# DaehwanKimLab/hisat-genotype

Hardware: AMD Instinct MI355X
Metric: typed reads/sec at HLA-A (~7k alleles, 2x150bp) (higher is better)
Workload: dtype u64 bitsets, f64 EM

## Files before the change

### hisat-genotype_amd/csrc/hgx_common.hpp

```cpp
#pragma once
#include <hip/hip_runtime.h>

#include <cstdint>
#include <cstring>
#include <cstdio>
#include <mutex>
#include <string>
#include <vector>

#include "hgx.h"

extern "C" void hgx_set_error(const char *fmt, ...);
extern "C" const char *hgx_test_switch(const char *name);
static inline bool hgx_switch_has(const char *name, const char *token) {
    const char *v = hgx_test_switch(name);
    if (!v) return false;
    const size_t n = strlen(token);
    for (const char *p = v;;) {
        const char *e = strchr(p, ',');
        const size_t len = e ? (size_t)(e - p) : strlen(p);
        if (len == n && memcmp(p, token, n) == 0) return true;
        if (!e) return false;
        p = e + 1;
    }
// ... 32 lines not shown
    uint64_t *d_exon_mask, *d_gene_mask;
    int pat_state = 0;
    uint16_t *d_pid = nullptr;
    uint32_t *d_vals = nullptr;
    int32_t *d_nval = nullptr;
    int pat_dmax = 0;
    std::mutex *pat_mu = nullptr;
};
#define HGX_PAT_D 512

struct hgx_classes {
    int32_t n_classes, a_pad, w64, c64;
    uint64_t *d_bits;
    int64_t *d_count;
    int64_t *d_first_row;
    uint64_t *d_bitsT;
    int32_t n_act = -1, a1p = 0;
    int32_t *d_act = nullptr;
    uint64_t *d_bitsC = nullptr;
    uint64_t *d_bitsTC = nullptr;
    int32_t *h_act = nullptr;
    int32_t *h_rank = nullptr;
    uint64_t *d_wrow = nullptr, *d_wcol = nullptr;
    void *d_setup0 = nullptr, *d_setup1 = nullptr;
    hipStream_t made_on = nullptr;
    hipEvent_t ready = nullptr;
    void *d_keep[12] = {nullptr, nullptr, nullptr, nullptr, nullptr, nullptr, nullptr, nullptr,
                        nullptr, nullptr, nullptr, nullptr};
};

// ... 55 lines not shown

int hgx_ensure_transposed(hgx_classes *c, hipStream_t st);
int hgx_pair_classes_sel(const hgx_index *ix, const uint64_t *compat, const int32_t *pair_off, const uint32_t *refs,
                         const int64_t *sel, int32_t n_pairs, uint64_t *eb, uint64_t *gb, uint64_t *eh,
                         uint64_t *gh, hipStream_t st);

struct hgx_groups;
int hgx_group_pairs_seg(hgx_groups **out, const int32_t *pair_off, const uint32_t *refs, int32_t n_pairs, int32_t level,
                        const uint32_t *pair_seg, void *stream);
int hgx_level_classes_grouped_seg(hgx_classes **out, const hgx_index *ix, const uint64_t *compat, const int32_t *pair_off,
                                  const uint32_t *refs, hgx_groups *g, uint64_t *rows_scratch, uint64_t *hash_scratch,
                                  const uint32_t *pair_seg, void *stream);
int hgx_dedup_classes_seg(hgx_classes **out, const uint64_t *rows, const uint64_t *row_hash, int64_t n_rows, int32_t a_pad,
                          const uint32_t *row_seg, void *stream);

int hgx_pair_classes_fused_launch(const hgx_index *ix, const uint64_t *compat, const int32_t *pair_off, const uint32_t *refs,
                                  int32_t n_pairs, int32_t level, unsigned long long *keys, uint32_t tmask, uint32_t *rep,
                                  uint32_t *slot_of, int *bad, uint64_t *rows, hipStream_t st);

int hgx_scan_u32_dev(const uint32_t *in, uint32_t *out, long n, void *scratch, uint32_t *total_dev, hipStream_t st);
size_t hgx_scan_u32_scratch_bytes(long n);
void hgx_front_set_last(int route, int decline, long long bytes);

int hgx_pair_classes_dedup_ev(hgx_classes **out, const hgx_index *ix, const uint64_t *compat, const int32_t *pair_off, const uint32_t *refs,
                              int32_t n_pairs, int32_t level, uint64_t *rows_scratch, void *stream, void *ev_begin, void *ev_end);

#define HGX_EMPTY_KEY 0xFFFFFFFFFFFFFFFFull

__device__ __forceinline__ uint64_t mix64(uint64_t x) {
    x ^= x >> 30; x *= 0xbf58476d1ce4e5b9ull;
// ... 70 lines not shown
```

### hisat-genotype_amd/csrc/hgx_counts.hip

```cpp
#include <algorithm>
#include <cstdint>
#include <vector>

#include <hip/hip_runtime.h>

#include "hgx_common.hpp"

namespace {
__device__ __forceinline__ uint64_t lane_u64(uint64_t v, int l) {
    return ((uint64_t)(uint32_t)__builtin_amdgcn_readlane((int)(v >> 32), l) << 32) | (uint32_t)__builtin_amdgcn_readlane((int)v, l);
}
}

__global__ __launch_bounds__(256) void k_first_set_rows(const uint64_t *__restrict__ BT, int n_rows, int c64, int32_t *__restrict__ first) {
    const int lane = threadIdx.x & 63;
    const long row = ((long)blockIdx.x * blockDim.x + threadIdx.x) >> 6;
    if (row >= n_rows) return;
    int best = 0x7fffffff;
    for (int w0 = 0; w0 < c64; w0 += 64) {
        const int w = w0 + lane;
        const uint64_t x = w < c64 ? BT[(size_t)row * c64 + w] : 0ull;
        const uint64_t hit = __ballot(x != 0ull);
        if (hit) {
            const int l = __builtin_ctzll(hit);
// ... 35 lines not shown
    hipStream_t st = (hipStream_t)stream;
    DevBuf b_a, b_f;
    ALLOC(b_a, (size_t)n * 4); ALLOC(b_f, (size_t)n * 4);
    { int rc_ = hgx_h2d(b_a.p, alleles_host, (size_t)n * 4, st); if (rc_) return rc_; }
    hipLaunchKernelGGL(k_first_classes, dim3(n), dim3(256), 0, st, c->d_bits, c->n_classes, c->w64, b_a.as<int32_t>(), b_f.as<int32_t>());
    HIPCHK(hipGetLastError());
    { int rc_ = hgx_d2h(first_host, b_f.p, (size_t)n * 4, st); if (rc_) return rc_; }
    { int rc_ = hgx_sync(st); if (rc_) return rc_; }
    return HGX_OK;
}

constexpr int AC_WAVES = 4;
__global__ __launch_bounds__(64 * AC_WAVES) void k_allele_counts_direct(const uint64_t *__restrict__ bits, int C, int w64,
                                                                         const int64_t *__restrict__ count, int per_wave,
                                                                         unsigned long long *__restrict__ cnt_part,
                                                                         int *__restrict__ first_part, int A) {
    __shared__ int s_first[AC_WAVES][32][64];
    __shared__ uint32_t s_cnt[AC_WAVES][32][64];
    const int lane = threadIdx.x & 63, wv = threadIdx.x >> 6;
    const int n_half = 2 * w64;
    const int hw = blockIdx.x * 64 + lane;
    const bool live = hw < n_half;
    const int c0 = (blockIdx.y * AC_WAVES + wv) * per_wave, c1 = min(C, c0 + per_wave);
    const uint32_t *rows = (const uint32_t *)bits;
    uint32_t acc[32];
#pragma unroll
    for (int b = 0; b < 32; ++b) { acc[b] = 0u; s_first[wv][b][lane] = 0x7fffffff; }
    uint32_t seen = 0u;
    constexpr int U = 8;
    uint32_t xn[U], nn[U];
    auto fetch = [&](int cb) {
#pragma unroll
        for (int u = 0; u < U; ++u) {
            const int c = cb + u;
            xn[u] = (live && c < c1) ? rows[(size_t)c * n_half + hw] : 0u;
            nn[u] = c < c1 ? (uint32_t)count[c] : 0u;
        }
    };
// ... 20 lines not shown
            }
        }
    }
#pragma unroll
    for (int b = 0; b < 32; ++b) s_cnt[wv][b][lane] = acc[b];
    __syncthreads();
    if (live) {
#pragma unroll
        for (int k = 0; k < 32 / AC_WAVES; ++k) {
            const int b = wv * (32 / AC_WAVES) + k;
            unsigned long long t = 0ull;
            int f = 0x7fffffff;
#pragma unroll
            for (int q = 0; q < AC_WAVES; ++q) { t += (unsigned long long)s_cnt[q][b][lane]; f = min(f, s_first[q][b][lane]); }
            const int a = hw * 32 + b;
            cnt_part[(size_t)blockIdx.y * A + a] = t;
            first_part[(size_t)blockIdx.y * A + a] = f;
        }
    }
}
__global__ void k_allele_counts_reduce(const unsigned long long *__restrict__ cnt_part, const int *__restrict__ first_part, int groups,
                                       int A, int64_t *__restrict__ cnt, int *__restrict__ first) {
    const int a = blockIdx.x * blockDim.x + threadIdx.x;
    if (a >= A) return;
    unsigned long long t = 0ull;
    int f = 0x7fffffff;
    for (int g0 = 0; g0 < groups; g0 += 8) {
        unsigned long long tv[8];
        int fv[8];
#pragma unroll
        for (int k = 0; k < 8; ++k) {
            const bool in = g0 + k < groups;
// ... 33 lines not shown
            m &= m - 1;
            if (cls >= n_classes) break;
            sum += count[cls];
            if (first < 0) first = cls;
        }
    }
    out_count[a] = sum;
    out_first[a] = first;
}

extern "C" int hgx_allele_counts_on(const hgx_classes *cc, int64_t *count_host, int32_t *first_host, void *stream);
extern "C" int hgx_allele_counts(const hgx_classes *cc, int64_t *count_host, int32_t *first_host) {
    return hgx_allele_counts_on(cc, count_host, first_host, nullptr);
}
extern "C" int hgx_allele_counts_on(const hgx_classes *cc, int64_t *count_host, int32_t *first_host, void *stream) {
    ARGCHK(cc && count_host && first_host);
    hipStream_t st = (hipStream_t)stream;
    hgx_classes_order_after(cc, st);
    hgx_classes *c = const_cast<hgx_classes *>(cc);
    const int A = c->a_pad;
    if (c->n_classes == 0) {
        for (int a = 0; a < A; ++a) { count_host[a] = 0; first_host[a] = -1; }
        return HGX_OK;
    }
    {
        const int C = c->n_classes;
        DevBuf b_cnt, b_first, b_big, b_cp, b_fp;
        ALLOC(b_cnt, (size_t)A * 8); ALLOC(b_first, (size_t)A * 4); ALLOC(b_big, 16);
        HIPCHK(hipMemsetAsync(b_big.p, 0, 16, st));
        hipLaunchKernelGGL(k_allele_counts_check, dim3(nblk(C, 256 * 16)), dim3(256), 0, st, c->d_count, C, b_big.as<unsigned long long>());
        const int spans = (2 * c->w64 + 63) / 64;
        const int groups = std::max(1, std::min(256 / std::max(spans, 1), (C + 64 * AC_WAVES - 1) / (64 * AC_WAVES)));
        const int per_wave = (C + groups * AC_WAVES - 1) / (groups * AC_WAVES);
        ALLOC(b_cp, (size_t)groups * A * 8); ALLOC(b_fp, (size_t)groups * A * 4);
        hipLaunchKernelGGL(k_allele_counts_direct, dim3(spans, groups), dim3(64 * AC_WAVES), 0, st, c->d_bits, C, c->w64, c->d_count,
                           per_wave, b_cp.as<unsigned long long>(), b_fp.as<int>(), A);
        hipLaunchKernelGGL(k_allele_counts_reduce, dim3(nblk(A, 64)), dim3(64), 0, st, b_cp.as<unsigned long long>(), b_fp.as<int>(),
                           groups, A, b_cnt.as<int64_t>(), b_first.as<int>());
        HIPCHK(hipGetLastError());
        unsigned long long big[2] = {0, 0};
        { int rc_ = hgx_d2h(count_host, b_cnt.p, (size_t)A * 8, st); if (rc_) return rc_; }
        { int rc_ = hgx_d2h(first_host, b_first.p, (size_t)A * 4, st); if (rc_) return rc_; }
        { int rc_ = hgx_d2h(big, b_big.p, 16, st); if (rc_) return rc_; }
        { int rc_ = hgx_sync(st); if (rc_) return rc_; }
        if (!big[0] && big[1] < (1ull << 32)) return HGX_OK;
    }
    int rc = hgx_ensure_transposed(c, st);
    if (rc) return rc;
    DevBuf b_c, b_i;
    ALLOC(b_c, (size_t)A * 8); ALLOC(b_i, (size_t)A * 4);
    hipLaunchKernelGGL(k_allele_counts_wide, dim3(nblk(A, 256)), dim3(256), 0, st, c->d_bitsT, A, c->c64, c->n_classes, c->d_count,
// ... 9 lines not shown
```

### hisat-genotype_amd/csrc/hgx_dedup.hip

```cpp
#include <algorithm>
#include <vector>

#include "hgx_common.hpp"


__global__ __launch_bounds__(256) void k_hash_rows(const uint64_t *__restrict__ rows, long n_rows, int w64,
                                                   const uint64_t *__restrict__ mask, uint64_t *__restrict__ hash) {
    const int lane = threadIdx.x & 63;
    const long row = ((long)blockIdx.x * blockDim.x + threadIdx.x) >> 6;
    if (row >= n_rows) return;
    uint64_t h = 0;
    bool nz = false;
    for (int w = lane; w < w64; w += 64) {
        uint64_t x = rows[(size_t)row * w64 + w];
        if (mask) x &= mask[w];
        h += word_hash(x, w);
        nz = nz || x != 0;
    }
    h = wave_sum_u64(h);
    const bool any_nz = __any(nz);
    if (lane == 0) hash[row] = finish_hash(h, any_nz);
}

#define SCAN_T 1024
// ... 132 lines not shown
        h = (h + 1) & tmask;
    }
}

__device__ __forceinline__ uint64_t readlane_u64(uint64_t v, int l) {
    const uint32_t lo = (uint32_t)__builtin_amdgcn_readlane((int)v, l), hi = (uint32_t)__builtin_amdgcn_readlane((int)(v >> 32), l);
    return ((uint64_t)hi << 32) | lo;
}
__device__ __forceinline__ uint64_t shfl_u64(uint64_t v, int l) {
    const uint32_t lo = __shfl((uint32_t)v, l, 64), hi = __shfl((uint32_t)(v >> 32), l, 64);
    return ((uint64_t)hi << 32) | lo;
}

template <int BS, int RPT>
__global__ __launch_bounds__(BS) void k_ht_insert(const uint64_t *__restrict__ hash, const int64_t *__restrict__ weight, long n,
                                                    unsigned long long *__restrict__ keys, uint32_t *__restrict__ first,
                                                    unsigned long long *__restrict__ cnt, uint32_t tmask,
                                                    uint32_t *__restrict__ slot_of) {
    constexpr int ROWS = BS * RPT, SLOTS = 2 * ROWS, SPT = SLOTS / BS;
    __shared__ unsigned long long lkey[SLOTS], lcnt[SLOTS];
    __shared__ uint32_t lmin[SLOTS];
    __shared__ uint8_t wtab[BS / 64][256];
    const int tid = threadIdx.x, lane = tid & 63;
    for (int s = tid; s < SLOTS; s += BS) { lkey[s] = HGX_EMPTY_KEY; lcnt[s] = 0; lmin[s] = HT_NONE; }
    const long base = (long)blockIdx.x * ROWS;
    uint64_t key[RPT];
    unsigned long long w[RPT];
#pragma unroll
    for (int r = 0; r < RPT; ++r) {
        const long i = base + (long)r * BS + tid;
        key[r] = i < n ? hash[i] : HGX_EMPTY_KEY;
        w[r] = weight && i < n ? (unsigned long long)weight[i] : 1ull;
    }
    __syncthreads();
    volatile uint8_t *wt = wtab[tid >> 6];
    uint32_t ls[RPT];
#pragma unroll
    for (int r = 0; r < RPT; ++r) {
        const bool valid = key[r] != HGX_EMPTY_KEY;
        const uint32_t bucket = (uint32_t)(key[r] >> 24) & 255u;
// ... 85 lines not shown
                          uint32_t *__restrict__ is_first) {
    const long s = (long)blockIdx.x * blockDim.x + threadIdx.x;
    if (s < T && keys[s] != HGX_EMPTY_KEY) is_first[first[s]] = 1u;
}
__global__ void k_ht_finalize(const unsigned long long *__restrict__ keys, const uint32_t *__restrict__ first,
                              const unsigned long long *__restrict__ cnt, long T, const uint32_t *__restrict__ rank,
                              int64_t *__restrict__ out_first, int64_t *__restrict__ out_count) {
    const long s = (long)blockIdx.x * blockDim.x + threadIdx.x;
    if (s >= T || keys[s] == HGX_EMPTY_KEY) return;
    const uint32_t c = rank[first[s]];
    out_first[c] = (int64_t)first[s];
    out_count[c] = (int64_t)cnt[s];
}
__global__ __launch_bounds__(256) void k_verify_ht(const uint64_t *__restrict__ rows, int w64, const uint64_t *__restrict__ mask,
                                                   const uint32_t *__restrict__ slot_of, const uint32_t *__restrict__ first, long n,
                                                   uint32_t *__restrict__ is_first,
                                                   int *__restrict__ bad, uint32_t *__restrict__ bad_rows = nullptr,
                                                   uint32_t *__restrict__ n_bad = nullptr, const uint32_t *__restrict__ seg = nullptr) {
    constexpr int R = 4;
    const int lane = threadIdx.x & 63;
    const long r0 = (((long)blockIdx.x * blockDim.x + threadIdx.x) >> 6) * R;
    if (r0 >= n) return;
    uint32_t sl[R], h[R];
#pragma unroll
    for (int k = 0; k < R; ++k) sl[k] = r0 + k < n ? slot_of[r0 + k] : HT_NONE;
#pragma unroll
    for (int k = 0; k < R; ++k) h[k] = sl[k] != HT_NONE ? first[sl[k]] : 0u;
    if (lane < R && r0 + lane < n) {
        uint32_t fl = 0;
#pragma unroll
        for (int k = 0; k < R; ++k)
            if (lane == k) fl = sl[k] != HT_NONE && h[k] == (uint32_t)(r0 + k) ? 1u : 0u;
        is_first[r0 + lane] = fl;
    }
    typedef unsigned long long u64x2 __attribute__((ext_vector_type(2)));
    const u64x2 *m = (const u64x2 *)mask;
// ... 108 lines not shown

__global__ void k_salt_keys(const uint64_t *__restrict__ in, const uint32_t *__restrict__ seg, long n, uint64_t *__restrict__ out) {
    const long i = (long)blockIdx.x * blockDim.x + threadIdx.x;
    if (i >= n) return;
    uint64_t k = in[i];
    if (k != HGX_EMPTY_KEY) {
        k = mix64(k ^ (0xd6e8feb86659fd93ull * (uint64_t)(seg[i] + 1u)));
        if (k == HGX_EMPTY_KEY) k = HGX_EMPTY_KEY - 1;
    }
    out[i] = k;
}

static hgx_classes *new_classes(int32_t a_pad);
static int dedup_hash_table(hgx_classes *cl, const uint64_t *rows, const uint64_t *keys_in, const int64_t *row_weight, long n,
                            int w64, const uint64_t *and_mask, hipStream_t st, bool small_blocks = false,
                            const uint32_t *seg = nullptr) {
    long T = 1024;
    while (T < 2 * n) T <<= 1;
    DevBuf b_keys, b_first, b_cnt, b_slot, b_flag, b_rank, b_tmp, b_meta, b_bad, b_salted;
    if (seg) {
        ALLOC(b_salted, (size_t)n * 8);
        hipLaunchKernelGGL(k_salt_keys, dim3(nblk(n, 256)), dim3(256), 0, st, keys_in, seg, n, b_salted.as<uint64_t>());
        keys_in = b_salted.as<uint64_t>();
    }
    ALLOC(b_keys, (size_t)T * 8); ALLOC(b_first, (size_t)T * 4); ALLOC(b_cnt, (size_t)T * 8);
    ALLOC(b_slot, (size_t)n * 4); ALLOC(b_flag, (size_t)n * 4); ALLOC(b_rank, (size_t)n * 4); ALLOC(b_meta, 16);
    ALLOC(b_bad, (size_t)n * 4);
    ALLOC(b_tmp, scan_scratch_bytes(n));
    auto number_classes = [&](bool scratch_is_zero) -> int {
        hipLaunchKernelGGL(k_ht_mark, dim3(nblk(T, 256)), dim3(256), 0, st, b_keys.as<unsigned long long>(), b_first.as<uint32_t>(), T,
                           b_flag.as<uint32_t>());
// ... 24 lines not shown
        }
        HIPCHK(hipMemsetAsync(b_flag.p, 0, (size_t)n * 4, st));
        { int rc_ = number_classes(false); if (rc_) return rc_; }
        HIPCHK(hipGetLastError());
        { int rc_ = hgx_d2h(meta, b_meta.p, 16, st); if (rc_) return rc_; }
        { int rc_ = hgx_sync(st); if (rc_) return rc_; }
        return HGX_OK;
    };
    cl->d_count = (decltype(cl->d_count))hgx_pool_alloc((size_t)n * 8);
    cl->d_first_row = (decltype(cl->d_first_row))hgx_pool_alloc((size_t)n * 8);
    if (!cl->d_count || !cl->d_first_row) { hgx_set_error("device allocation failed"); return HGX_ENOMEM; }
    hipLaunchKernelGGL(k_ht_init, dim3(nblk(T, 256)), dim3(256), 0, st, b_keys.as<unsigned long long>(),
                       b_first.as<uint32_t>(), b_cnt.as<unsigned long long>(), T, b_meta.as<uint32_t>(),
                       b_tmp.as<unsigned long long>(), (long)(scan_scratch_bytes(n) / 8));
    if (small_blocks)
        hipLaunchKernelGGL((k_ht_insert<256, 4>), dim3(nblk(n, 1024)), dim3(256), 0, st, keys_in, row_weight, n, b_keys.as<unsigned long long>(),
                           b_first.as<uint32_t>(), b_cnt.as<unsigned long long>(), (uint32_t)(T - 1), b_slot.as<uint32_t>());
    else
        hipLaunchKernelGGL((k_ht_insert<1024, 1>), dim3(nblk(n, 1024)), dim3(1024), 0, st, keys_in, row_weight, n, b_keys.as<unsigned long long>(),
                           b_first.as<uint32_t>(), b_cnt.as<unsigned long long>(), (uint32_t)(T - 1), b_slot.as<uint32_t>());
    hipLaunchKernelGGL(k_verify_ht, dim3(nblk((n + 3) / 4, 4)), dim3(256), 0, st, rows, w64, and_mask, b_slot.as<uint32_t>(),
                       b_first.as<uint32_t>(), n, b_flag.as<uint32_t>(), b_meta.as<int>(), b_bad.as<uint32_t>(), b_meta.as<uint32_t>() + 2, seg);
    { int rc_ = scan_classes(b_flag.as<uint32_t>(), b_rank.as<uint32_t>(), n, b_tmp.p, b_meta.as<uint32_t>() + 1,
                             ScanFin{b_slot.as<uint32_t>(), b_cnt.as<unsigned long long>(), cl->d_first_row, cl->d_count}, st); if (rc_) return rc_; }
    auto finalize_again = [&]() {
        hipLaunchKernelGGL(k_ht_finalize, dim3(nblk(T, 256)), dim3(256), 0, st, b_keys.as<unsigned long long>(), b_first.as<uint32_t>(),
                           b_cnt.as<unsigned long long>(), T, b_rank.as<uint32_t>(), cl->d_first_row, cl->d_count);
    };
    const bool one_trip = n <= 65536;
    int n_alloc = (int)n;
    if (!one_trip) {
        { int rc_ = hgx_d2h(meta, b_meta.p, 16, st); if (rc_) return rc_; }
        { int rc_ = hgx_sync(st); if (rc_) return rc_; }
        HIPCHK(hipGetLastError());
        if (meta[2]) { int rc_ = resolve_collisions(); if (rc_) return rc_; finalize_again(); }
        n_alloc = (int)meta[1];
        if (n_alloc == 0) return HGX_OK;
    }
    cl->d_bits = (decltype(cl->d_bits))hgx_pool_alloc((size_t)n_alloc * w64 * 8);
    if (!cl->d_bits) { hgx_set_error("device allocation failed"); return HGX_ENOMEM; }
    if (one_trip)
        hipLaunchKernelGGL(k_ht_gather_slots, dim3(nblk(T, 4)), dim3(256), 0, st, rows, w64, and_mask, b_keys.as<unsigned long long>(),
                           b_first.as<uint32_t>(), b_rank.as<uint32_t>(), T, cl->d_bits);
    else
        hipLaunchKernelGGL(k_ht_gather, dim3(nblk(n_alloc, 4)), dim3(256), 0, st, rows, w64, and_mask, cl->d_first_row, n_alloc, cl->d_bits);
    HIPCHK(hipGetLastError());
    if (one_trip) {
        { int rc_ = hgx_d2h(meta, b_meta.p, 16, st); if (rc_) return rc_; }
        { int rc_ = hgx_sync(st); if (rc_) return rc_; }
        if (meta[2]) {
            { int rc_ = resolve_collisions(); if (rc_) return rc_; }
            finalize_again();
            hipLaunchKernelGGL(k_ht_gather_slots, dim3(nblk(T, 4)), dim3(256), 0, st, rows, w64, and_mask, b_keys.as<unsigned long long>(),
                               b_first.as<uint32_t>(), b_rank.as<uint32_t>(), T, cl->d_bits);
            HIPCHK(hipGetLastError());
            { int rc_ = hgx_sync(st); if (rc_) return rc_; }
        }
    } else {
        cl->made_on = st;
        if (hipEventCreateWithFlags(&cl->ready, hipEventDisableTiming) == hipSuccess) (void)hipEventRecord(cl->ready, st);
// ... 3 lines not shown
    const int n_runs = (int)meta[1];
    cl->n_classes = n_runs;
    return HGX_OK;
}

template <class T, class Destroy> static int fail_clean(int rc, T **out, hipStream_t st, Destroy destroy) {
    if (rc != HGX_OK && out && *out) {
        (void)hipStreamSynchronize(st);
        destroy(*out);
        *out = nullptr;
    }
    return rc;
}

static int dedup_classes_impl(hgx_classes **out, const uint64_t *rows, const uint64_t *row_hash, const int64_t *row_weight,
                              int64_t n_rows, int32_t a_pad, const uint64_t *and_mask, void *stream, const uint32_t *seg = nullptr) {
    ARGCHK(out && n_rows >= 0 && a_pad > 0 && a_pad % 512 == 0);
    ARGCHK(n_rows < (1ll << 31));
    hipStream_t st = (hipStream_t)stream;
    const int w64 = a_pad / 64;
    hgx_classes *cl = new_classes(a_pad);
    *out = cl;
    if (n_rows == 0) return HGX_OK;
    ARGCHK(rows);
    const long n = n_rows;
    DevBuf b_hash;
    const uint64_t *keys_in = row_hash;
    if (!row_hash || and_mask) {
        ALLOC(b_hash, n * 8);
        hipLaunchKernelGGL(k_hash_rows, dim3(nblk(n, 4)), dim3(256), 0, st, rows, n, w64, and_mask, b_hash.as<uint64_t>());
        keys_in = b_hash.as<uint64_t>();
    }
    return dedup_hash_table(cl, rows, keys_in, row_weight, n, w64, and_mask, st, false, seg);
}

struct HtInit { unsigned long long *keys; uint32_t *first; unsigned long long *cnt; long T; uint32_t *meta;
                unsigned long long *scan_state; long n_state; };
__global__ void k_sig_keys(const int32_t *__restrict__ pair_off, const uint32_t *__restrict__ refs, int n_pairs, uint32_t level,
                           uint64_t *__restrict__ key, const uint32_t *__restrict__ seg, HtInit init) {
    const long p = (long)blockIdx.x * blockDim.x + threadIdx.x;
    for (long s = p; s < init.T; s += (long)gridDim.x * blockDim.x) { init.keys[s] = HGX_EMPTY_KEY; init.first[s] = HT_NONE; init.cnt[s] = 0; }
    if (p < 4) init.meta[p] = 0;
    if (p < init.n_state) init.scan_state[p] = 0;
    if (p >= n_pairs) return;
    uint64_t h = 0x243f6a8885a308d3ull;
    uint32_t cnt = 0;
    for (int r = pair_off[p]; r < pair_off[p + 1]; ++r) {
        const uint32_t x = refs[r];
// ... 88 lines not shown
    g->d_first = (int64_t *)hgx_pool_alloc((size_t)n * 8);
    g->d_count = (int64_t *)hgx_pool_alloc((size_t)n * 8);
    if (!g->d_first || !g->d_count) { hgx_set_error("device allocation failed"); return HGX_ENOMEM; }
    long T = 1024;
    while (T < 2 * n) T <<= 1;
    DevBuf b_key, b_keys, b_first, b_cnt, b_slot, b_flag, b_rank, b_tmp, b_meta;
    ALLOC(b_key, (size_t)n * 8);
    ALLOC(b_keys, (size_t)T * 8); ALLOC(b_first, (size_t)T * 4); ALLOC(b_cnt, (size_t)T * 8);
    ALLOC(b_slot, (size_t)n * 4); ALLOC(b_flag, (size_t)n * 4); ALLOC(b_rank, (size_t)n * 4); ALLOC(b_meta, 16);
    ALLOC(b_tmp, scan_scratch_bytes(n));
    const HtInit init{b_keys.as<unsigned long long>(), b_first.as<uint32_t>(), b_cnt.as<unsigned long long>(), T,
                      b_meta.as<uint32_t>(), b_tmp.as<unsigned long long>(), (long)(scan_scratch_bytes(n) / 8)};
    hipLaunchKernelGGL(k_sig_keys, dim3(nblk(std::max<long>(n, 1024), 256)), dim3(256), 0, st, pair_off, refs, n_pairs, (uint32_t)level, b_key.as<uint64_t>(),
                       seg, init);
    hipLaunchKernelGGL((k_ht_insert<256, 4>), dim3(nblk(n, 1024)), dim3(256), 0, st, b_key.as<uint64_t>(), (const int64_t *)nullptr, n,
                       b_keys.as<unsigned long long>(), b_first.as<uint32_t>(), b_cnt.as<unsigned long long>(), (uint32_t)(T - 1),
                       b_slot.as<uint32_t>());
    hipLaunchKernelGGL(k_sig_verify, dim3(nblk(n, 256)), dim3(256), 0, st, pair_off, refs, n_pairs, (uint32_t)level,
                       b_slot.as<uint32_t>(), b_first.as<uint32_t>(), b_flag.as<uint32_t>(), b_meta.as<int>(), seg);
    { int rc_ = scan_classes(b_flag.as<uint32_t>(), b_rank.as<uint32_t>(), n, b_tmp.p, b_meta.as<uint32_t>() + 1,
                             ScanFin{b_slot.as<uint32_t>(), b_cnt.as<unsigned long long>(), g->d_first, g->d_count}, st); if (rc_) return rc_; }
    HIPCHK(hipGetLastError());
    { int rc_ = hgx_d2h(g->meta, b_meta.p, 16, st); if (rc_) return rc_; }
    DevBuf *keep[] = {&b_key, &b_keys, &b_first, &b_cnt, &b_slot, &b_flag, &b_rank, &b_tmp, &b_meta};
    for (int i = 0; i < 9; ++i) { g->scratch[i] = keep[i]->p; keep[i]->p = nullptr; }
    g->finished = false;
    return HGX_OK;
}

extern "C" int hgx_group_pairs(hgx_groups **out, const int32_t *pair_off, const uint32_t *refs, int32_t n_pairs, int32_t level,
                               void *stream) {
// ... 83 lines not shown
        g->d_first = nullptr; g->d_count = nullptr;
    }
    hgx_groups_destroy(g);
    return rc;
}

extern "C" int hgx_classes_destroy(hgx_classes *c);
int hgx_dedup_classes_seg(hgx_classes **out, const uint64_t *rows, const uint64_t *row_hash, int64_t n_rows, int32_t a_pad,
                          const uint32_t *row_seg, void *stream) {
    if (out) *out = nullptr;
    return fail_clean(dedup_classes_impl(out, rows, row_hash, nullptr, n_rows, a_pad, nullptr, stream, row_seg), out, (hipStream_t)stream,
                      hgx_classes_destroy);
}
extern "C" int hgx_dedup_classes(hgx_classes **out, const uint64_t *rows, const uint64_t *row_hash, const int64_t *row_weight,
                                 int64_t n_rows, int32_t a_pad, const uint64_t *and_mask, void *stream) {
    if (out) *out = nullptr;
    return fail_clean(dedup_classes_impl(out, rows, row_hash, row_weight, n_rows, a_pad, and_mask, stream), out, (hipStream_t)stream,
                      hgx_classes_destroy);
}

#ifdef HGX_LAB
#include "lab/hgx_fused_dedup_lab.inc"
#else
extern "C" int hgx_pair_classes_dedup(hgx_classes **out, const hgx_index *, const uint64_t *, const int32_t *, const uint32_t *, int32_t, int32_t,
                                      uint64_t *, void *) {
    if (out) *out = nullptr;
    hgx_set_error("hgx_pair_classes_dedup is lab code (measured slower than hgx_pair_classes + hgx_dedup_classes): build libhgx_lab.so");
    return HGX_EINVAL;
}
#endif

extern "C" int hgx_classes_destroy(hgx_classes *c) {
    if (!c) return HGX_OK;
// ... 81 lines not shown
```

### hisat-genotype_amd/csrc/hgx_type.hip

```cpp
#include <hip/hip_runtime.h>

#include <algorithm>
#include <array>
#include <atomic>
#include <chrono>
#include <cmath>
#include <cstdlib>
#include <cstring>
#include <map>
#include <mutex>
#include <numeric>
#include <string>
#include <thread>
#include <vector>

#include "hgx_common.hpp"
#include "hgx_emx.hpp"
#include "hgx_internal.hpp"

extern "C" int hgx_em_set_fast(int on);
int em_tie_prefix_scope(int on);
int em_fast_mode();
void em_count_rerun();
extern "C" int hgx_em_last_order(int32_t *order_host, int32_t n);
// ... 108 lines not shown
        if (stamps[2] < stamps[1] && stamps[0] < stamps[3]) return false;
    }
    return true;
}
static int ss_class_of(DevStreams &D, hipStream_t s) {
    if (D.reps.empty()) return -1;
    const double alone = ss_chain_us(D, s, nullptr, 2);
    for (size_t c = 0; c < D.reps.size(); ++c) {
        double beside = ss_chain_us(D, s, D.reps[c], 1);
        if (beside > 1.25 * alone && beside < 1.9 * alone) beside = std::min(beside, ss_chain_us(D, s, D.reps[c], 2));
        if (beside > 1.5 * alone) return (int)c;
    }
    return -1;
}
static int make_gene_stream(hipStream_t *out, int least) {
    const char *gcu = getenv("HGX_GENE_CUS");
    const int n_gene_cus = gcu ? atoi(gcu) : 0;
    if (n_gene_cus > 0 && n_gene_cus < 256) {
        uint32_t mask[8] = {0, 0, 0, 0, 0, 0, 0, 0};
        for (int b = 0; b < n_gene_cus; ++b) mask[b >> 5] |= 1u << (b & 31);
        HIPCHK(hipExtStreamCreateWithCUMask(out, 8, mask));
    } else
        HIPCHK(hipStreamCreateWithPriority(out, hipStreamNonBlocking, least));
    return HGX_OK;
}
static int make_stream_set(int dev, DevStreams &D, StreamSet &set) {
    const auto t0 = std::chrono::steady_clock::now();
    int least = 0, greatest = 0;
    HIPCHK(hipDeviceGetStreamPriorityRange(&least, &greatest));
    const bool probe = !hgx_switch_has("streams", "unplaced");
    set = StreamSet();
    set.dev = dev;
    std::vector<hipStream_t> spare;
    struct Spare { std::vector<hipStream_t> &v; ~Spare() { for (hipStream_t x : v) (void)hipStreamDestroy(x); } } spare_guard{spare};
    auto keep_class = [&](hipStream_t s, int cls) -> int {
        if (cls >= 0) return cls;
        D.reps.push_back(s);
        D.em_in_class.push_back(0);
// ... 76 lines not shown
}
bool hgx_ss_forget_stream(void *stream) {
    std::lock_guard<std::mutex> g(g_ss_mu);
    for (auto &kv : g_ss) {
        DevStreams &D = kv.second;
        auto it = D.caller_cls.find((hipStream_t)stream);
        if (it == D.caller_cls.end()) continue;
        if (D.caller_in_class[(size_t)it->second] > 0) D.caller_in_class[(size_t)it->second]--;
        D.caller_cls.erase(it);
        for (hipStream_t r : D.reps) if (r == (hipStream_t)stream) return true;
        return false;
    }
    return false;
}
namespace {
int acquire_streams(StreamSet &s) {
    int dev = 0;
    HIPCHK(hipGetDevice(&dev));
    std::lock_guard<std::mutex> g(g_ss_mu);
    DevStreams &D = g_ss[dev];
    if (!D.free.empty()) { s = D.free.front(); D.free.erase(D.free.begin()); return HGX_OK; }
    StreamSet made;
    const int rc = make_stream_set(dev, D, made);
    if (rc) {
        if (made.em) (void)hipStreamDestroy(made.em);
        if (made.gene) (void)hipStreamDestroy(made.gene);
        if (made.fork) (void)hipEventDestroy(made.fork);
        return rc;
    }
    s = made;
    return HGX_OK;
}
void release_streams(const StreamSet &s) {
    if (s.dev < 0) return;
    std::lock_guard<std::mutex> g(g_ss_mu);
    DevStreams &D = g_ss[s.dev];
    auto it = D.free.begin();
    while (it != D.free.end() && it->id < s.id) ++it;
    D.free.insert(it, s);
}

struct GateHold {
    hgx_gate *g = nullptr;
    explicit GateHold(hgx_gate *gate) : g(gate) { if (g) g->mu.lock(); }
    void release() { if (g) { g->mu.unlock(); g = nullptr; } }
    ~GateHold() { release(); }
};

double now_s() { return std::chrono::duration<double>(std::chrono::steady_clock::now().time_since_epoch()).count(); }

inline int em_mode_one(int em_fast) { return em_fast == 2 ? 0 : em_fast; }
inline int em_mode_many(int em_fast) { return em_fast == 0 ? 1 : (em_fast == 2 ? 0 : em_fast); }

struct EmFastScope {
// ... 87 lines not shown
}

extern "C" int hgx_gate_create(hgx_gate **g) { ARGCHK(g); *g = new hgx_gate(); return HGX_OK; }
extern "C" int hgx_gate_destroy(hgx_gate *g) { delete g; return HGX_OK; }

namespace {

struct GeneSide {
    hgx_classes *gcl = nullptr;
    std::vector<int32_t> counted;
    std::vector<int64_t> cnt;
    int rc = HGX_OK;
    char err[512] = "";
};

int gene_rank(hgx_classes *gcl, int32_t A, int32_t a_pad, hipStream_t st, GeneSide &g);

int gene_side(const hgx_index *ix, const hgx_dbatch *db, const uint64_t *compat, uint64_t *gene_bits, uint64_t *gene_hash,
              bool rows_ready, const hgx_type_opts *opts, hipStream_t st, GeneSide &g) {
    int32_t A = 0, a_pad = 0;
    int rc = hgx_index_dims(ix, &A, &a_pad, nullptr, nullptr);
    if (rc) return rc;
#ifdef HGX_LAB
    if (!rows_ready && hgx_test_switch("fused")) {
        rc = hgx_pair_classes_dedup_ev(&g.gcl, ix, compat, db->d_pair_off, db->d_pair_ref, db->n_pairs, HGX_LEVEL_GENE, gene_bits, st,
                                       opts->ev_pairs_begin, opts->ev_pairs_end);
        if (rc == HGX_OK) return gene_rank(g.gcl, A, a_pad, st, g);
        if (rc != HGX_ECOLLISION) return rc;
    }
#endif
    if (!rows_ready) {
        if (opts->ev_pairs_begin) HIPCHK(hipEventRecord((hipEvent_t)opts->ev_pairs_begin, st));
        rc = hgx_pair_classes(ix, compat, db->d_pair_off, db->d_pair_ref, db->n_pairs, nullptr, gene_bits, nullptr, gene_hash, st);
        if (rc) return rc;
        if (opts->ev_pairs_end) HIPCHK(hipEventRecord((hipEvent_t)opts->ev_pairs_end, st));
    }
    rc = hgx_dedup_classes(&g.gcl, gene_bits, gene_hash, nullptr, db->n_pairs, a_pad, nullptr, st);
    if (rc) return rc;
    return gene_rank(g.gcl, A, a_pad, st, g);
}

int gene_rank(hgx_classes *gcl, int32_t A, int32_t a_pad, hipStream_t st, GeneSide &g) {
    int rc;
    std::vector<int64_t> cnt((size_t)a_pad);
    std::vector<int32_t> first((size_t)a_pad);
    rc = hgx_allele_counts_on(gcl, cnt.data(), first.data(), st);
    if (rc) return rc;
    int32_t C = 0;
    hgx_classes_dims(gcl, &C, nullptr);
    std::vector<int64_t> fr((size_t)std::max(C, 1));
    rc = hgx_classes_to_host(gcl, nullptr, nullptr, fr.data());
    if (rc) return rc;
    g.cnt.assign(cnt.begin(), cnt.begin() + A);
    for (int32_t a = 0; a < A; ++a) if (cnt[a] > 0) g.counted.push_back(a);
    std::sort(g.counted.begin(), g.counted.end(), [&](int32_t a, int32_t b) {
        if (cnt[a] != cnt[b]) return cnt[a] > cnt[b];
        const int64_t ia = fr[first[a]], ib = fr[first[b]];
        if (ia != ib) return ia < ib;
        return a < b;
    });
    return HGX_OK;
// ... 223 lines not shown
    const bool prof = getenv("HGX_TYPE_PROFILE") != nullptr;
    const double tq0 = now_s();
    double tq1 = tq0;

    if (overlap) {
        em_stream = ss.em;
        gene_stream = ss.gene;
        HIPCHK(hipEventRecord(ss.fork, stream));
        HIPCHK(hipStreamWaitEvent(gene_stream, ss.fork, 0));
        if (by_list) {
            rc = hgx_group_pairs(&groups, db->d_pair_off, db->d_pair_ref, n_pairs, HGX_LEVEL_EXON, em_stream);
            if (rc) return rc;
        }
        int dev = 0;
        HIPCHK(hipGetDevice(&dev));
        worker = std::thread([&, dev] {
            if (hipSetDevice(dev) != hipSuccess) { gs.rc = HGX_EHIP; snprintf(gs.err, sizeof(gs.err), "hipSetDevice failed on the gene-side thread"); return; }
            gs.rc = gene_side(ix, db, compat, b_gbits.as<uint64_t>(), b_ghash.as<uint64_t>(), rows_ready, opts, gene_stream, gs);
            if (gs.rc) snprintf(gs.err, sizeof(gs.err), "%s", hgx_last_error());
        });
        if (groups) {
            int64_t ng = 0;
            rc = hgx_groups_dims(groups, &ng, nullptr);
            if (rc) return rc;
        }
        tq1 = now_s();
        HIPCHK(hipStreamWaitEvent(em_stream, ss.fork, 0));
    } else {
        gs.rc = gene_side(ix, db, compat, b_gbits.as<uint64_t>(), b_ghash.as<uint64_t>(), rows_ready, opts, stream, gs);
        if (gs.rc) return gs.rc;
    }
    auto finish_gene = [&]() -> int {
        if (worker.joinable()) worker.join();
        if (gs.rc) { hgx_set_error("%s", gs.err[0] ? gs.err : "gene-level side failed"); return gs.rc; }
        t->counted = gs.counted;
        t->cnt = gs.cnt;
        return HGX_OK;
    };

    if (hla) {
        if (by_list) {
            if (groups) rc = hgx_level_classes_grouped(&ecl, ix, compat, db->d_pair_off, db->d_pair_ref, groups, b_ebits.as<uint64_t>(),
                                                       b_ehash.as<uint64_t>(), em_stream);
            else rc = hgx_level_classes(&ecl, ix, compat, db->d_pair_off, db->d_pair_ref, n_pairs, HGX_LEVEL_EXON, b_ebits.as<uint64_t>(),
// ... 122 lines not shown

extern "C" int hgx_type_classes(hgx_typing **out, const hgx_locus *loc, hgx_classes *exon_cl, hgx_classes *gene_cl, int32_t n_reads,
                                int32_t n_pairs, const hgx_type_opts *opts, void *stream) {
    ARGCHK(out && loc && gene_cl && opts);
    *out = nullptr;
    const bool hla = loc->base_kind == HGX_BASE_HLA;
    ARGCHK(!hla || exon_cl);
    ARGCHK(gene_cl->a_pad == loc->a_pad && (!exon_cl || exon_cl->a_pad == loc->a_pad));
    ARGCHK((int32_t)loc->name_rank.size() == loc->A && (int32_t)loc->allele_len.size() == loc->A);
    hgx_typing *t = new hgx_typing();
    t->n_reads = n_reads; t->n_pairs = n_pairs; t->n_alleles = loc->A;
    if (n_reads <= 0) { *out = t; return HGX_OK; }
    hipStream_t st = (hipStream_t)stream;
    EmFastScope em_mode(em_mode_one(opts->em_fast));
    GeneSide gs;
    int rc = gene_rank(gene_cl, loc->A, loc->a_pad, st, gs);
    if (!rc) {
        t->counted = gs.counted;
        t->cnt = gs.cnt;
        if (hla) rc = finish_hla(t, loc, exon_cl, opts, st, st, [&](hgx_classes **g) { *g = gene_cl; return HGX_OK; });
        else rc = finish_other(t, loc, gene_cl, st);
    }
    if (rc) { delete t; return rc; }
    *out = t;
    return HGX_OK;
}

extern "C" int hgx_type_batch(hgx_typing **out, const hgx_locus *loc, const hgx_index *ix, const hgx_batch *batch,
                              const hgx_type_opts *opts, void *stream) {
    ARGCHK(out && batch);
    *out = nullptr;
// ... 717 lines not shown
```

Before: 499.5 million.

## Slice gene-side dedup and count kernels into smaller launches beside EM

Splits the gene-level hash insert, verify, gather and allele-count kernels into several smaller launches when the gene side runs on its own thread next to the exon EM work and only one stream set is in use. The goal is to keep the big gene-side kernels from filling the GPU for long stretches, so EM-stream kernels can interleave and the two sides overlap better. It also removes the HGX_GENE_CUS CU-mask stream option. In exchange it adds launch overhead and per-slice tail effects, and it introduces a global counter of stream sets in use.

Result: faster. 520.5 million, median of 6 (+4.2%).

```diff
diff --git a/hisat-genotype_amd/csrc/hgx_common.hpp b/hisat-genotype_amd/csrc/hgx_common.hpp
--- a/hisat-genotype_amd/csrc/hgx_common.hpp
+++ b/hisat-genotype_amd/csrc/hgx_common.hpp
@@ -70,6 +70,7 @@
     uint64_t *d_bits;
     int64_t *d_count;
     int64_t *d_first_row;
+    int64_t n_rows_in = 0;
     uint64_t *d_bitsT;
     int32_t n_act = -1, a1p = 0;
     int32_t *d_act = nullptr;
@@ -155,6 +156,22 @@
 int hgx_dedup_classes_seg(hgx_classes **out, const uint64_t *rows, const uint64_t *row_hash, int64_t n_rows, int32_t a_pad,
                           const uint32_t *row_seg, void *stream);
 
+enum { HGX_SLICE_INSERT = 0, HGX_SLICE_VERIFY = 1, HGX_SLICE_GATHER = 2, HGX_SLICE_COUNTS = 3 };
+enum { HGX_SLICES_NEVER = 0,
+       HGX_SLICES_IF_FORCED = 1,
+       HGX_SLICES_BESIDE_EM = 2 };
+int hgx_gene_slices(int kernel, long n_rows, int use);
+template <class F> static inline void hgx_for_slices(long W, int slices, F fn) {
+    const long S = slices < 1 ? 1 : ((long)slices < W ? (long)slices : (W > 0 ? W : 1));
+    for (long k = 0; k < S; ++k) {
+        const long g0 = k * W / S, g1 = (k + 1) * W / S;
+        if (g1 > g0) fn(g0, g1 - g0);
+    }
+}
+int hgx_dedup_classes_sliced(hgx_classes **out, const uint64_t *rows, const uint64_t *row_hash, const int64_t *row_weight,
+                             int64_t n_rows, int32_t a_pad, const uint64_t *and_mask, void *stream, int slice_use);
+int hgx_allele_counts_sliced(const hgx_classes *cc, int64_t *count_host, int32_t *first_host, void *stream, int slice_use);
+
 int hgx_pair_classes_fused_launch(const hgx_index *ix, const uint64_t *compat, const int32_t *pair_off, const uint32_t *refs,
                                   int32_t n_pairs, int32_t level, unsigned long long *keys, uint32_t tmask, uint32_t *rep,
                                   uint32_t *slot_of, int *bad, uint64_t *rows, hipStream_t st);
diff --git a/hisat-genotype_amd/csrc/hgx_counts.hip b/hisat-genotype_amd/csrc/hgx_counts.hip
--- a/hisat-genotype_amd/csrc/hgx_counts.hip
+++ b/hisat-genotype_amd/csrc/hgx_counts.hip
@@ -73,14 +73,15 @@
 __global__ __launch_bounds__(64 * AC_WAVES) void k_allele_counts_direct(const uint64_t *__restrict__ bits, int C, int w64,
                                                                          const int64_t *__restrict__ count, int per_wave,
                                                                          unsigned long long *__restrict__ cnt_part,
-                                                                         int *__restrict__ first_part, int A) {
+                                                                         int *__restrict__ first_part, int A, int class0, int group0) {
     __shared__ int s_first[AC_WAVES][32][64];
     __shared__ uint32_t s_cnt[AC_WAVES][32][64];
     const int lane = threadIdx.x & 63, wv = threadIdx.x >> 6;
     const int n_half = 2 * w64;
     const int hw = blockIdx.x * 64 + lane;
     const bool live = hw < n_half;
-    const int c0 = (blockIdx.y * AC_WAVES + wv) * per_wave, c1 = min(C, c0 + per_wave);
+    const int c0 = min(C, class0 + (blockIdx.y * AC_WAVES + wv) * per_wave), c1 = min(C, c0 + per_wave);
+    const size_t part = (size_t)(group0 + blockIdx.y) * A;
     const uint32_t *rows = (const uint32_t *)bits;
     uint32_t acc[32];
 #pragma unroll
@@ -131,8 +132,8 @@
 #pragma unroll
             for (int q = 0; q < AC_WAVES; ++q) { t += (unsigned long long)s_cnt[q][b][lane]; f = min(f, s_first[q][b][lane]); }
             const int a = hw * 32 + b;
-            cnt_part[(size_t)blockIdx.y * A + a] = t;
-            first_part[(size_t)blockIdx.y * A + a] = f;
+            cnt_part[part + a] = t;
+            first_part[part + a] = f;
         }
     }
 }
@@ -196,6 +197,9 @@
     return hgx_allele_counts_on(cc, count_host, first_host, nullptr);
 }
 extern "C" int hgx_allele_counts_on(const hgx_classes *cc, int64_t *count_host, int32_t *first_host, void *stream) {
+    return hgx_allele_counts_sliced(cc, count_host, first_host, stream, HGX_SLICES_IF_FORCED);
+}
+int hgx_allele_counts_sliced(const hgx_classes *cc, int64_t *count_host, int32_t *first_host, void *stream, int slice_use) {
     ARGCHK(cc && count_host && first_host);
     hipStream_t st = (hipStream_t)stream;
     hgx_classes_order_after(cc, st);
@@ -212,11 +216,24 @@
         HIPCHK(hipMemsetAsync(b_big.p, 0, 16, st));
         hipLaunchKernelGGL(k_allele_counts_check, dim3(nblk(C, 256 * 16)), dim3(256), 0, st, c->d_count, C, b_big.as<unsigned long long>());
         const int spans = (2 * c->w64 + 63) / 64;
-        const int groups = std::max(1, std::min(256 / std::max(spans, 1), (C + 64 * AC_WAVES - 1) / (64 * AC_WAVES)));
-        const int per_wave = (C + groups * AC_WAVES - 1) / (groups * AC_WAVES);
+        const int wg_classes = 64 * AC_WAVES;
+        auto groups_for = [&](long n_cls) {
+            return (int)std::max(1L, std::min((long)(256 / std::max(spans, 1)), (n_cls + wg_classes - 1) / wg_classes));
+        };
+        const int slices = hgx_gene_slices(HGX_SLICE_COUNTS, (long)c->n_rows_in, slice_use);
+        int groups = 0;
+        hgx_for_slices(nblk(C, wg_classes), slices, [&](long g0, long ng) {
+            groups += groups_for(std::min((long)C, (g0 + ng) * wg_classes) - g0 * wg_classes);
+        });
         ALLOC(b_cp, (size_t)groups * A * 8); ALLOC(b_fp, (size_t)groups * A * 4);
-        hipLaunchKernelGGL(k_allele_counts_direct, dim3(spans, groups), dim3(64 * AC_WAVES), 0, st, c->d_bits, C, c->w64, c->d_count,
-                           per_wave, b_cp.as<unsigned long long>(), b_fp.as<int>(), A);
+        int group0 = 0;
+        hgx_for_slices(nblk(C, wg_classes), slices, [&](long g0, long ng) {
+            const int lo = (int)(g0 * wg_classes), hi = (int)std::min((long)C, (g0 + ng) * wg_classes);
+            const int gs = groups_for(hi - lo), per_wave = (hi - lo + gs * AC_WAVES - 1) / (gs * AC_WAVES);
+            hipLaunchKernelGGL(k_allele_counts_direct, dim3(spans, gs), dim3(64 * AC_WAVES), 0, st, c->d_bits, hi, c->w64, c->d_count,
+                               per_wave, b_cp.as<unsigned long long>(), b_fp.as<int>(), A, lo, group0);
+            group0 += gs;
+        });
         hipLaunchKernelGGL(k_allele_counts_reduce, dim3(nblk(A, 64)), dim3(64), 0, st, b_cp.as<unsigned long long>(), b_fp.as<int>(),
                            groups, A, b_cnt.as<int64_t>(), b_first.as<int>());
         HIPCHK(hipGetLastError());
diff --git a/hisat-genotype_amd/csrc/hgx_dedup.hip b/hisat-genotype_amd/csrc/hgx_dedup.hip
--- a/hisat-genotype_amd/csrc/hgx_dedup.hip
+++ b/hisat-genotype_amd/csrc/hgx_dedup.hip
@@ -170,7 +170,7 @@
 
 template <int BS, int RPT>
 __global__ __launch_bounds__(BS) void k_ht_insert(const uint64_t *__restrict__ hash, const int64_t *__restrict__ weight, long n,
-                                                    unsigned long long *__restrict__ keys, uint32_t *__restrict__ first,
+                                                    long row0, unsigned long long *__restrict__ keys, uint32_t *__restrict__ first,
                                                     unsigned long long *__restrict__ cnt, uint32_t tmask,
                                                     uint32_t *__restrict__ slot_of) {
     constexpr int ROWS = BS * RPT, SLOTS = 2 * ROWS, SPT = SLOTS / BS;
@@ -179,7 +179,7 @@
     __shared__ uint8_t wtab[BS / 64][256];
     const int tid = threadIdx.x, lane = tid & 63;
     for (int s = tid; s < SLOTS; s += BS) { lkey[s] = HGX_EMPTY_KEY; lcnt[s] = 0; lmin[s] = HT_NONE; }
-    const long base = (long)blockIdx.x * ROWS;
+    const long base = row0 + (long)blockIdx.x * ROWS;
     uint64_t key[RPT];
     unsigned long long w[RPT];
 #pragma unroll
@@ -295,12 +295,12 @@
 }
 __global__ __launch_bounds__(256) void k_verify_ht(const uint64_t *__restrict__ rows, int w64, const uint64_t *__restrict__ mask,
                                                    const uint32_t *__restrict__ slot_of, const uint32_t *__restrict__ first, long n,
-                                                   uint32_t *__restrict__ is_first,
+                                                   long row0, uint32_t *__restrict__ is_first,
                                                    int *__restrict__ bad, uint32_t *__restrict__ bad_rows = nullptr,
                                                    uint32_t *__restrict__ n_bad = nullptr, const uint32_t *__restrict__ seg = nullptr) {
     constexpr int R = 4;
     const int lane = threadIdx.x & 63;
-    const long r0 = (((long)blockIdx.x * blockDim.x + threadIdx.x) >> 6) * R;
+    const long r0 = row0 + (((long)blockIdx.x * blockDim.x + threadIdx.x) >> 6) * R;
     if (r0 >= n) return;
     uint32_t sl[R], h[R];
 #pragma unroll
@@ -439,7 +439,8 @@
 static hgx_classes *new_classes(int32_t a_pad);
 static int dedup_hash_table(hgx_classes *cl, const uint64_t *rows, const uint64_t *keys_in, const int64_t *row_weight, long n,
                             int w64, const uint64_t *and_mask, hipStream_t st, bool small_blocks = false,
-                            const uint32_t *seg = nullptr) {
+                            const uint32_t *seg = nullptr, int slice_use = HGX_SLICES_NEVER) {
+    cl->n_rows_in = n;
     long T = 1024;
     while (T < 2 * n) T <<= 1;
     DevBuf b_keys, b_first, b_cnt, b_slot, b_flag, b_rank, b_tmp, b_meta, b_bad, b_salted;
@@ -494,13 +495,19 @@
                        b_first.as<uint32_t>(), b_cnt.as<unsigned long long>(), T, b_meta.as<uint32_t>(),
                        b_tmp.as<unsigned long long>(), (long)(scan_scratch_bytes(n) / 8));
     if (small_blocks)
-        hipLaunchKernelGGL((k_ht_insert<256, 4>), dim3(nblk(n, 1024)), dim3(256), 0, st, keys_in, row_weight, n, b_keys.as<unsigned long long>(),
+        hipLaunchKernelGGL((k_ht_insert<256, 4>), dim3(nblk(n, 1024)), dim3(256), 0, st, keys_in, row_weight, n, 0L, b_keys.as<unsigned long long>(),
                            b_first.as<uint32_t>(), b_cnt.as<unsigned long long>(), (uint32_t)(T - 1), b_slot.as<uint32_t>());
     else
-        hipLaunchKernelGGL((k_ht_insert<1024, 1>), dim3(nblk(n, 1024)), dim3(1024), 0, st, keys_in, row_weight, n, b_keys.as<unsigned long long>(),
-                           b_first.as<uint32_t>(), b_cnt.as<unsigned long long>(), (uint32_t)(T - 1), b_slot.as<uint32_t>());
-    hipLaunchKernelGGL(k_verify_ht, dim3(nblk((n + 3) / 4, 4)), dim3(256), 0, st, rows, w64, and_mask, b_slot.as<uint32_t>(),
-                       b_first.as<uint32_t>(), n, b_flag.as<uint32_t>(), b_meta.as<int>(), b_bad.as<uint32_t>(), b_meta.as<uint32_t>() + 2, seg);
+        hgx_for_slices(nblk(n, 1024), hgx_gene_slices(HGX_SLICE_INSERT, n, slice_use), [&](long g0, long ng) {
+            hipLaunchKernelGGL((k_ht_insert<1024, 1>), dim3((unsigned)ng), dim3(1024), 0, st, keys_in, row_weight, std::min(n, (g0 + ng) * 1024),
+                               g0 * 1024, b_keys.as<unsigned long long>(), b_first.as<uint32_t>(), b_cnt.as<unsigned long long>(),
+                               (uint32_t)(T - 1), b_slot.as<uint32_t>());
+        });
+    hgx_for_slices(nblk(n, 16), hgx_gene_slices(HGX_SLICE_VERIFY, n, slice_use), [&](long g0, long ng) {
+        hipLaunchKernelGGL(k_verify_ht, dim3((unsigned)ng), dim3(256), 0, st, rows, w64, and_mask, b_slot.as<uint32_t>(), b_first.as<uint32_t>(),
+                           std::min(n, (g0 + ng) * 16), g0 * 16, b_flag.as<uint32_t>(), b_meta.as<int>(), b_bad.as<uint32_t>(),
+                           b_meta.as<uint32_t>() + 2, seg);
+    });
     { int rc_ = scan_classes(b_flag.as<uint32_t>(), b_rank.as<uint32_t>(), n, b_tmp.p, b_meta.as<uint32_t>() + 1,
                              ScanFin{b_slot.as<uint32_t>(), b_cnt.as<unsigned long long>(), cl->d_first_row, cl->d_count}, st); if (rc_) return rc_; }
     auto finalize_again = [&]() {
@@ -523,7 +530,11 @@
         hipLaunchKernelGGL(k_ht_gather_slots, dim3(nblk(T, 4)), dim3(256), 0, st, rows, w64, and_mask, b_keys.as<unsigned long long>(),
                            b_first.as<uint32_t>(), b_rank.as<uint32_t>(), T, cl->d_bits);
     else
-        hipLaunchKernelGGL(k_ht_gather, dim3(nblk(n_alloc, 4)), dim3(256), 0, st, rows, w64, and_mask, cl->d_first_row, n_alloc, cl->d_bits);
+        hgx_for_slices(nblk(n_alloc, 4), hgx_gene_slices(HGX_SLICE_GATHER, n, slice_use), [&](long g0, long ng) {
+            const long c0 = g0 * 4, c1 = std::min((long)n_alloc, (g0 + ng) * 4);
+            hipLaunchKernelGGL(k_ht_gather, dim3((unsigned)ng), dim3(256), 0, st, rows, w64, and_mask, cl->d_first_row + c0, (int)(c1 - c0),
+                               cl->d_bits + (size_t)c0 * w64);
+        });
     HIPCHK(hipGetLastError());
     if (one_trip) {
         { int rc_ = hgx_d2h(meta, b_meta.p, 16, st); if (rc_) return rc_; }
@@ -557,7 +568,8 @@
 }
 
 static int dedup_classes_impl(hgx_classes **out, const uint64_t *rows, const uint64_t *row_hash, const int64_t *row_weight,
-                              int64_t n_rows, int32_t a_pad, const uint64_t *and_mask, void *stream, const uint32_t *seg = nullptr) {
+                              int64_t n_rows, int32_t a_pad, const uint64_t *and_mask, void *stream, const uint32_t *seg = nullptr,
+                              int slice_use = HGX_SLICES_NEVER) {
     ARGCHK(out && n_rows >= 0 && a_pad > 0 && a_pad % 512 == 0);
     ARGCHK(n_rows < (1ll << 31));
     hipStream_t st = (hipStream_t)stream;
@@ -574,7 +586,24 @@
         hipLaunchKernelGGL(k_hash_rows, dim3(nblk(n, 4)), dim3(256), 0, st, rows, n, w64, and_mask, b_hash.as<uint64_t>());
         keys_in = b_hash.as<uint64_t>();
     }
-    return dedup_hash_table(cl, rows, keys_in, row_weight, n, w64, and_mask, st, false, seg);
+    return dedup_hash_table(cl, rows, keys_in, row_weight, n, w64, and_mask, st, false, seg, slice_use);
+}
+
+constexpr long GENE_SLICE_MIN_ROWS = 131072;
+constexpr long GENE_SLICE_ROWS = 50000;
+int hgx_gene_slices(int kernel, long n_rows, int use) {
+    if (use == HGX_SLICES_NEVER) return 1;
+    if (const char *sw = hgx_test_switch("gene_slices")) return std::max(1, atoi(sw));
+    if (use != HGX_SLICES_BESIDE_EM) return 1;
+    long nv = 1;
+    if (const char *sw = hgx_test_switch("gene_slices_verify")) {
+        int each[4];
+        if (sscanf(sw, "%d,%d,%d,%d", &each[0], &each[1], &each[2], &each[3]) == 4) return std::max(1, each[kernel]);
+        nv = std::max(1, atoi(sw));
+    }
+    else if (GENE_SLICE_ROWS > 0 && n_rows >= GENE_SLICE_MIN_ROWS) nv = std::min(32L, (n_rows + GENE_SLICE_ROWS - 1) / GENE_SLICE_ROWS);
+    static const long share[4] = {36, 120, 12, 24};
+    return (int)std::max(1L, (nv * share[kernel] + share[HGX_SLICE_VERIFY] / 2) / share[HGX_SLICE_VERIFY]);
 }
 
 struct HtInit { unsigned long long *keys; uint32_t *first; unsigned long long *cnt; long T; uint32_t *meta;
@@ -693,7 +722,7 @@
     hipLaunchKernelGGL(k_sig_keys, dim3(nblk(std::max<long>(n, 1024), 256)), dim3(256), 0, st, pair_off, refs, n_pairs, (uint32_t)level, b_key.as<uint64_t>(),
                        seg, init);
     hipLaunchKernelGGL((k_ht_insert<256, 4>), dim3(nblk(n, 1024)), dim3(256), 0, st, b_key.as<uint64_t>(), (const int64_t *)nullptr, n,
-                       b_keys.as<unsigned long long>(), b_first.as<uint32_t>(), b_cnt.as<unsigned long long>(), (uint32_t)(T - 1),
+                       0L, b_keys.as<unsigned long long>(), b_first.as<uint32_t>(), b_cnt.as<unsigned long long>(), (uint32_t)(T - 1),
                        b_slot.as<uint32_t>());
     hipLaunchKernelGGL(k_sig_verify, dim3(nblk(n, 256)), dim3(256), 0, st, pair_off, refs, n_pairs, (uint32_t)level,
                        b_slot.as<uint32_t>(), b_first.as<uint32_t>(), b_flag.as<uint32_t>(), b_meta.as<int>(), seg);
@@ -807,9 +836,13 @@
 }
 extern "C" int hgx_dedup_classes(hgx_classes **out, const uint64_t *rows, const uint64_t *row_hash, const int64_t *row_weight,
                                  int64_t n_rows, int32_t a_pad, const uint64_t *and_mask, void *stream) {
+    return hgx_dedup_classes_sliced(out, rows, row_hash, row_weight, n_rows, a_pad, and_mask, stream, HGX_SLICES_IF_FORCED);
+}
+int hgx_dedup_classes_sliced(hgx_classes **out, const uint64_t *rows, const uint64_t *row_hash, const int64_t *row_weight,
+                             int64_t n_rows, int32_t a_pad, const uint64_t *and_mask, void *stream, int slice_use) {
     if (out) *out = nullptr;
-    return fail_clean(dedup_classes_impl(out, rows, row_hash, row_weight, n_rows, a_pad, and_mask, stream), out, (hipStream_t)stream,
-                      hgx_classes_destroy);
+    return fail_clean(dedup_classes_impl(out, rows, row_hash, row_weight, n_rows, a_pad, and_mask, stream, nullptr, slice_use), out,
+                      (hipStream_t)stream, hgx_classes_destroy);
 }
 
 #ifdef HGX_LAB
diff --git a/hisat-genotype_amd/csrc/hgx_type.hip b/hisat-genotype_amd/csrc/hgx_type.hip
--- a/hisat-genotype_amd/csrc/hgx_type.hip
+++ b/hisat-genotype_amd/csrc/hgx_type.hip
@@ -146,14 +146,7 @@
     return -1;
 }
 static int make_gene_stream(hipStream_t *out, int least) {
-    const char *gcu = getenv("HGX_GENE_CUS");
-    const int n_gene_cus = gcu ? atoi(gcu) : 0;
-    if (n_gene_cus > 0 && n_gene_cus < 256) {
-        uint32_t mask[8] = {0, 0, 0, 0, 0, 0, 0, 0};
-        for (int b = 0; b < n_gene_cus; ++b) mask[b >> 5] |= 1u << (b & 31);
-        HIPCHK(hipExtStreamCreateWithCUMask(out, 8, mask));
-    } else
-        HIPCHK(hipStreamCreateWithPriority(out, hipStreamNonBlocking, least));
+    HIPCHK(hipStreamCreateWithPriority(out, hipStreamNonBlocking, least));
     return HGX_OK;
 }
 static int make_stream_set(int dev, DevStreams &D, StreamSet &set) {
@@ -260,12 +253,15 @@
     return false;
 }
 namespace {
+std::atomic<int> g_sets_out[64];
 int acquire_streams(StreamSet &s) {
     int dev = 0;
     HIPCHK(hipGetDevice(&dev));
+    g_sets_out[dev & 63].fetch_add(1, std::memory_order_relaxed);
+    struct Uncount { int dev; bool armed; ~Uncount() { if (armed) g_sets_out[dev & 63].fetch_sub(1, std::memory_order_relaxed); } } uncount{dev, true};
     std::lock_guard<std::mutex> g(g_ss_mu);
     DevStreams &D = g_ss[dev];
-    if (!D.free.empty()) { s = D.free.front(); D.free.erase(D.free.begin()); return HGX_OK; }
+    if (!D.free.empty()) { s = D.free.front(); D.free.erase(D.free.begin()); uncount.armed = false; return HGX_OK; }
     StreamSet made;
     const int rc = make_stream_set(dev, D, made);
     if (rc) {
@@ -275,15 +271,23 @@
         return rc;
     }
     s = made;
+    uncount.armed = false;
     return HGX_OK;
 }
 void release_streams(const StreamSet &s) {
     if (s.dev < 0) return;
+    g_sets_out[s.dev & 63].fetch_sub(1, std::memory_order_relaxed);
     std::lock_guard<std::mutex> g(g_ss_mu);
     DevStreams &D = g_ss[s.dev];
     auto it = D.free.begin();
     while (it != D.free.end() && it->id < s.id) ++it;
     D.free.insert(it, s);
+}
+
+int stream_sets_in_use() {
+    int dev = 0;
+    if (hipGetDevice(&dev) != hipSuccess) return 1;
+    return g_sets_out[dev & 63].load(std::memory_order_relaxed);
 }
 
 struct GateHold {
@@ -401,10 +405,11 @@
     char err[512] = "";
 };
 
-int gene_rank(hgx_classes *gcl, int32_t A, int32_t a_pad, hipStream_t st, GeneSide &g);
+int gene_rank(hgx_classes *gcl, int32_t A, int32_t a_pad, hipStream_t st, GeneSide &g, int slice_use);
 
 int gene_side(const hgx_index *ix, const hgx_dbatch *db, const uint64_t *compat, uint64_t *gene_bits, uint64_t *gene_hash,
-              bool rows_ready, const hgx_type_opts *opts, hipStream_t st, GeneSide &g) {
+              bool rows_ready, const hgx_type_opts *opts, hipStream_t st, GeneSide &g, bool beside_em) {
+    const int slice_use = beside_em ? HGX_SLICES_BESIDE_EM : HGX_SLICES_IF_FORCED;
     int32_t A = 0, a_pad = 0;
     int rc = hgx_index_dims(ix, &A, &a_pad, nullptr, nullptr);
     if (rc) return rc;
@@ -412,7 +417,7 @@
     if (!rows_ready && hgx_test_switch("fused")) {
         rc = hgx_pair_classes_dedup_ev(&g.gcl, ix, compat, db->d_pair_off, db->d_pair_ref, db->n_pairs, HGX_LEVEL_GENE, gene_bits, st,
                                        opts->ev_pairs_begin, opts->ev_pairs_end);
-        if (rc == HGX_OK) return gene_rank(g.gcl, A, a_pad, st, g);
+        if (rc == HGX_OK) return gene_rank(g.gcl, A, a_pad, st, g, slice_use);
         if (rc != HGX_ECOLLISION) return rc;
     }
 #endif
@@ -422,16 +427,16 @@
         if (rc) return rc;
         if (opts->ev_pairs_end) HIPCHK(hipEventRecord((hipEvent_t)opts->ev_pairs_end, st));
     }
-    rc = hgx_dedup_classes(&g.gcl, gene_bits, gene_hash, nullptr, db->n_pairs, a_pad, nullptr, st);
-    if (rc) return rc;
-    return gene_rank(g.gcl, A, a_pad, st, g);
-}
-
-int gene_rank(hgx_classes *gcl, int32_t A, int32_t a_pad, hipStream_t st, GeneSide &g) {
+    rc = hgx_dedup_classes_sliced(&g.gcl, gene_bits, gene_hash, nullptr, db->n_pairs, a_pad, nullptr, st, slice_use);
+    if (rc) return rc;
+    return gene_rank(g.gcl, A, a_pad, st, g, slice_use);
+}
+
+int gene_rank(hgx_classes *gcl, int32_t A, int32_t a_pad, hipStream_t st, GeneSide &g, int slice_use) {
     int rc;
     std::vector<int64_t> cnt((size_t)a_pad);
     std::vector<int32_t> first((size_t)a_pad);
-    rc = hgx_allele_counts_on(gcl, cnt.data(), first.data(), st);
+    rc = hgx_allele_counts_sliced(gcl, cnt.data(), first.data(), st, slice_use);
     if (rc) return rc;
     int32_t C = 0;
     hgx_classes_dims(gcl, &C, nullptr);
@@ -685,9 +690,10 @@
         }
         int dev = 0;
         HIPCHK(hipGetDevice(&dev));
-        worker = std::thread([&, dev] {
+        const bool slices = stream_sets_in_use() <= 1;
+        worker = std::thread([&, dev, slices] {
             if (hipSetDevice(dev) != hipSuccess) { gs.rc = HGX_EHIP; snprintf(gs.err, sizeof(gs.err), "hipSetDevice failed on the gene-side thread"); return; }
-            gs.rc = gene_side(ix, db, compat, b_gbits.as<uint64_t>(), b_ghash.as<uint64_t>(), rows_ready, opts, gene_stream, gs);
+            gs.rc = gene_side(ix, db, compat, b_gbits.as<uint64_t>(), b_ghash.as<uint64_t>(), rows_ready, opts, gene_stream, gs, slices);
             if (gs.rc) snprintf(gs.err, sizeof(gs.err), "%s", hgx_last_error());
         });
         if (groups) {
@@ -698,7 +704,7 @@
         tq1 = now_s();
         HIPCHK(hipStreamWaitEvent(em_stream, ss.fork, 0));
     } else {
-        gs.rc = gene_side(ix, db, compat, b_gbits.as<uint64_t>(), b_ghash.as<uint64_t>(), rows_ready, opts, stream, gs);
+        gs.rc = gene_side(ix, db, compat, b_gbits.as<uint64_t>(), b_ghash.as<uint64_t>(), rows_ready, opts, stream, gs, false);
         if (gs.rc) return gs.rc;
     }
     auto finish_gene = [&]() -> int {
@@ -851,7 +857,7 @@
     hipStream_t st = (hipStream_t)stream;
     EmFastScope em_mode(em_mode_one(opts->em_fast));
     GeneSide gs;
-    int rc = gene_rank(gene_cl, loc->A, loc->a_pad, st, gs);
+    int rc = gene_rank(gene_cl, loc->A, loc->a_pad, st, gs, HGX_SLICES_IF_FORCED);
     if (!rc) {
         t->counted = gs.counted;
         t->cnt = gs.cnt;
```
